# alonbebchuk/GNN-Pretraining

Hardware: AMD Instinct MI355X
Metric: pretrain graphs/sec (s4 multi-task) (higher is better)
Workload: dtype fp32; 1 GPU; s4 (NFM+LP+NC+GC+GP) pre-training step, 4 domains x 8 synthetic ENZYMES-shaped graphs per rank (input dims 7/4/37/21, hidden 256, 5 GIN layers), PCGrad + clip + AdamW; global_batch_graphs=32, parallelism=dp1, setup_steps=30, full=False, index_rng=reference, index_draws=native (csrc_host/hostdraw.cpp), cross_stream_sync=gates, ranks=1, devices_visible=1

## Files before the change

gnn_pretraining_amd/csrc/gemm_f32.hip:

```cpp
#include <algorithm>
#include <cstdlib>
#include <cstring>
#include <type_traits>

#include "gnnmp_internal.h"

namespace {

using gmp::f32x16;

constexpr int BK_DEFAULT = 32;
constexpr int THREADS = 256;

template <int R, bool KMAJOR, int BK>
struct TileLoader {
    static constexpr int NV = R * BK / 4 / THREADS;
    float4 v[NV];

    __device__ __forceinline__ void load(const float* __restrict__ P, int64_t ld, int64_t r0, int64_t rtot, int64_t k0,
                                         int64_t K, bool vec, int t) {
#pragma unroll
        for (int s = 0; s < NV; ++s) {
            const int f = t + s * THREADS;
            float4 x = make_float4(0.f, 0.f, 0.f, 0.f);
// ... 243 lines not shown
                    if (g.accumulate) v += out[row * ldo + col];
                    if (EPI) {
                        if (g.resid) v += g.resid[row * g.ldr + col];
                        if (g.scale) v = v * sc + sh;
                    }
                    if (g.relu) v = fmaxf(v, 0.f);
                }
                out[row * ldo + col] = v;
            }
        }
}

__global__ __launch_bounds__(256) void splitk_reduce_kernel(GemmArgs g) {
    const int64_t total = g.M * g.N;
    for (int64_t i = (int64_t)blockIdx.x * 256 + threadIdx.x; i < total; i += (int64_t)gridDim.x * 256) {
        float s = 0.f;
        for (int z = 0; z < g.splitk; ++z) s += g.partial[(int64_t)z * total + i];
        const int64_t row = i / g.N, col = i % g.N;
        float v = g.alpha * s + (g.bias ? g.bias[col] : 0.f);
        if (g.accumulate) v += g.C[row * g.ldc + col];
        if (g.resid) v += g.resid[row * g.ldr + col];
        if (g.scale) v = v * g.scale[col] + g.shift[col];
        if (g.relu) v = fmaxf(v, 0.f);
        g.C[row * g.ldc + col] = v;
    }
}

template <bool VEC>
__global__ __launch_bounds__(256) void grouped_reduce_kernel(const GemmArgs g) {
    const int grp = blockIdx.y;
    const int64_t total = g.M * g.N;
    if (VEC) {
        const int64_t quads = total / 4, mq = (g.M + 3) / 4;
        for (int64_t q = (int64_t)blockIdx.x * 256 + threadIdx.x; q < quads + mq; q += (int64_t)gridDim.x * 256) {
            if (q < quads) {
                const float* base = g.gpart + (int64_t)grp * g.gsplit * total + 4 * q;
                float4 s = make_float4(0.f, 0.f, 0.f, 0.f);
                for (int z0 = 0; z0 < g.gsplit; z0 += 8) {
                    float4 v[8];
#pragma unroll
                    for (int u = 0; u < 8; ++u)
                        v[u] = z0 + u < g.gsplit ? *reinterpret_cast<const float4*>(base + (int64_t)(z0 + u) * total) : make_float4(0.f, 0.f, 0.f, 0.f);
#pragma unroll
                    for (int u = 0; u < 8; ++u)
                        if (z0 + u < g.gsplit) { s.x += v[u].x; s.y += v[u].y; s.z += v[u].z; s.w += v[u].w; }
                }
                const int64_t i = 4 * q;
                *reinterpret_cast<float4*>(g.C + g.coff[grp] + (i / g.N) * g.ldc + i % g.N) = make_float4(g.alpha * s.x, g.alpha * s.y, g.alpha * s.z, g.alpha * s.w);
            } else if (g.asum) {
                for (int64_t m = 4 * (q - quads); m < g.M && m < 4 * (q - quads) + 4; ++m) {
                    float s = 0.f;
                    for (int z = 0; z < g.gsplit; ++z) s += g.gasum_part[((int64_t)grp * g.gsplit + z) * g.M + m];
                    g.asum[g.asumoff[grp] + m] = s;
                }
            }
        }
        return;
    }
    for (int64_t i = (int64_t)blockIdx.x * 256 + threadIdx.x; i < total + g.M; i += (int64_t)gridDim.x * 256) {
        float s = 0.f;
        if (i < total) {
            for (int z = 0; z < g.gsplit; ++z) s += g.gpart[((int64_t)grp * g.gsplit + z) * total + i];
            g.C[g.coff[grp] + (i / g.N) * g.ldc + i % g.N] = g.alpha * s;
        } else if (g.asum) {
            const int64_t m = i - total;
            for (int z = 0; z < g.gsplit; ++z) s += g.gasum_part[((int64_t)grp * g.gsplit + z) * g.M + m];
            g.asum[g.asumoff[grp] + m] = s;
        }
    }
}

inline void launch_grouped_reduce(const GemmArgs& g, int groups, hipStream_t st) {
    bool vec = g.N % 4 == 0 && g.ldc % 4 == 0 && (((uintptr_t)g.C | (uintptr_t)g.gpart) & 15) == 0;
    for (int i = 0; i < groups && vec; ++i) vec = g.coff[i] % 4 == 0;
    if (vec) {
        const int blocks = (int)std::min<int64_t>((g.M * g.N / 4 + (g.M + 3) / 4 + 255) / 256, 256);
        hipLaunchKernelGGL(grouped_reduce_kernel<true>, dim3(blocks, groups), dim3(256), 0, st, g);
    } else {
        const int blocks = (int)std::min<int64_t>((g.M * g.N + g.M + 255) / 256, 256);
        hipLaunchKernelGGL(grouped_reduce_kernel<false>, dim3(blocks, groups), dim3(256), 0, st, g);
    }
}

constexpr int CS_ROWS = 256;
__global__ __launch_bounds__(256) void colsum_partial_kernel(const float* __restrict__ A, float* __restrict__ part,
                                                             int64_t M, int64_t N, int64_t lda) {
    __shared__ float sh[4][64];
    const int c = threadIdx.x % 64, rl = threadIdx.x / 64;
    const int64_t col = (int64_t)blockIdx.x * 64 + c;
    const int64_t r0 = (int64_t)blockIdx.y * CS_ROWS, r1 = r0 + CS_ROWS < M ? r0 + CS_ROWS : M;
    float s = 0.f;
    if (col < N)
        for (int64_t r = r0 + rl; r < r1; r += 4) s += A[r * lda + col];
    sh[rl][c] = s;
    __syncthreads();
    if (rl == 0 && col < N) part[(int64_t)blockIdx.y * N + col] = (sh[0][c] + sh[1][c]) + (sh[2][c] + sh[3][c]);
}
__global__ __launch_bounds__(256) void colsum_final_kernel(const float* __restrict__ part, float* __restrict__ out,
                                                           int64_t nparts, int64_t N, int accumulate) {
    const int64_t col = (int64_t)blockIdx.x * 256 + threadIdx.x;
    if (col >= N) return;
    float s = 0.f;
    for (int64_t p = 0; p < nparts; ++p) s += part[p * N + col];
    out[col] = accumulate ? out[col] + s : s;
}

inline bool aligned16(const void* p) { return ((uintptr_t)p & 15) == 0; }

template <int BK>
bool fast_ok(int mode, const GemmArgs& g, int64_t min_rows) {
    if (!g.vecA || !g.vecB) return false;
    if (mode == GMP_GEMM_NT) return g.K % BK == 0 && g.K > 0 && min_rows >= 1 && g.N >= 1;
    if (mode == GMP_GEMM_NN) return g.K % BK == 0 && g.K > 0 && min_rows >= 1 && g.N % 4 == 0 && g.N >= 4;
    return g.M % 4 == 0 && g.M >= 4 && g.N % 4 == 0 && g.N >= 4;
}

template <int BM, int BN, int BK = BK_DEFAULT>
void launch_mode(int mode, const GemmArgs& g, dim3 grid, hipStream_t st, bool fast = false) {
#define GMP_GEMM_LAUNCH(AK, BKM)                                                                                    \
    do {                                                                                                           \
        if (fast) hipLaunchKernelGGL((gemm_kernel<BM, BN, AK, BKM, BK, true>), grid, dim3(THREADS), 0, st, g);      \
        else hipLaunchKernelGGL((gemm_kernel<BM, BN, AK, BKM, BK, false>), grid, dim3(THREADS), 0, st, g);          \
    } while (0)
    switch (mode) {
        case GMP_GEMM_NT:
            if (g.scale || g.resid) {
                if (fast) hipLaunchKernelGGL((gemm_kernel<BM, BN, false, false, BK, true, true>), grid, dim3(THREADS), 0, st, g);
                else hipLaunchKernelGGL((gemm_kernel<BM, BN, false, false, BK, false, true>), grid, dim3(THREADS), 0, st, g);
                break;
            }
            GMP_GEMM_LAUNCH(false, false);
            break;
        case GMP_GEMM_NN: GMP_GEMM_LAUNCH(false, true); break;
        default:          GMP_GEMM_LAUNCH(true, true); break;
    }
#undef GMP_GEMM_LAUNCH
}

constexpr int PIPE_TILES[4][2] = {{2, 2}, {1, 2}, {2, 1}, {1, 1}};

template <int TM, int TN, bool A_KC, bool B_KC, int STAGES, int BUFS = STAGES, bool EPI = false>
int launch_pipe_cfg(const GemmArgs& g, int tiles_m, int tiles_n, int z, hipStream_t st) {
    if constexpr (!EPI && A_KC && B_KC) {
        if (g.scale || g.resid) return launch_pipe_cfg<TM, TN, A_KC, B_KC, STAGES, BUFS, true>(g, tiles_m, tiles_n, z, st);
    }
    using C = g2::Cfg<TM, TN, A_KC, B_KC, STAGES, BUFS>;
    auto kern = g2::gemm_pipe_kernel<TM, TN, A_KC, B_KC, STAGES, BUFS, EPI>;
    static std::atomic<uint64_t> attr_set{0};
    if (int rc = gmp::reserve_lds(attr_set, reinterpret_cast<const void*>(kern), C::LDS_BYTES, "gemm_pipe")) return rc;
    hipLaunchKernelGGL(kern, dim3((unsigned)(tiles_m * tiles_n), 1, (unsigned)z), dim3(g2::THREADS), C::LDS_BYTES, st, g, tiles_m, tiles_n);
    return gmp::check_launch("gemm_pipe_kernel");
}

template <bool KC, int GEN>
int launch_pipe_gen(const GemmArgs& g, int64_t rows, int z, hipStream_t st) {
    using C = g2::Cfg<1, 1, KC, KC, 4, 4>;
    auto kern = g2::gemm_pipe_kernel<1, 1, KC, KC, 4, 4, false, GEN>;
    static std::atomic<uint64_t> attr_set{0};
    if (int rc = gmp::reserve_lds(attr_set, reinterpret_cast<const void*>(kern), C::LDS_BYTES, "gemm_pipe (generated operand)")) return rc;
    const int tiles_m = (int)((rows + 63) / 64), tiles_n = (int)((g.N + 63) / 64);
    hipLaunchKernelGGL(kern, dim3((unsigned)(tiles_m * tiles_n), 1, (unsigned)z), dim3(g2::THREADS), C::LDS_BYTES, st, g, tiles_m, tiles_n);
    return gmp::check_launch("gemm_pipe_kernel (generated operand)");
}

template <bool A_KC, bool B_KC>
int launch_pipe_tile(int tile, const GemmArgs& g, int64_t rows, int z, hipStream_t st) {
    const int TMs = PIPE_TILES[tile][0], TNs = PIPE_TILES[tile][1];
    const int tiles_m = (int)((rows + 64 * TMs - 1) / (64 * TMs)), tiles_n = (int)((g.N + 64 * TNs - 1) / (64 * TNs));
    const char* e = getenv("GMP_GEMM_PIPE_STAGES");
    const int deep = e ? atoi(e) : 0;
    switch (tile) {
        case 0: return launch_pipe_cfg<2, 2, A_KC, B_KC, 4>(g, tiles_m, tiles_n, z, st);
        case 1: return deep == 3 ? launch_pipe_cfg<1, 2, A_KC, B_KC, 3>(g, tiles_m, tiles_n, z, st)
                                 : launch_pipe_cfg<1, 2, A_KC, B_KC, 4>(g, tiles_m, tiles_n, z, st);
        case 2: return deep == 3 ? launch_pipe_cfg<2, 1, A_KC, B_KC, 3>(g, tiles_m, tiles_n, z, st)
                                 : launch_pipe_cfg<2, 1, A_KC, B_KC, 4>(g, tiles_m, tiles_n, z, st);
        default: return deep == 3 ? launch_pipe_cfg<1, 1, A_KC, B_KC, 3>(g, tiles_m, tiles_n, z, st)
                      : deep == 32 ? launch_pipe_cfg<1, 1, A_KC, B_KC, 3, 2>(g, tiles_m, tiles_n, z, st)
                                   : launch_pipe_cfg<1, 1, A_KC, B_KC, 4>(g, tiles_m, tiles_n, z, st);
    }
}

int launch_pipe(int mode, int tile, const GemmArgs& g_in, int64_t rows, int z, hipStream_t st) {
    const GemmArgs& g = g_in;
    if (mode == GMP_GEMM_NT) return launch_pipe_tile<true, true>(tile, g, rows, z, st);
    if (mode == GMP_GEMM_NN) return launch_pipe_tile<true, false>(tile, g, rows, z, st);
    return launch_pipe_tile<false, false>(tile, g, rows, z, st);
}

inline bool pipe_enabled() {
    const char* e = getenv("GMP_GEMM_IMPL");
    return !(e && !strcmp(e, "old"));
}
inline int64_t pipe_min_rows() { return 1024; }
inline int pipe_forced_tile() {
    const char* e = getenv("GMP_GEMM_PIPE_TILE");
    return e ? atoi(e) : -1;
}

int pipe_pick_tile(int64_t rows, int64_t N, int64_t z) {
    (void)rows; (void)N; (void)z;
    if (pipe_forced_tile() >= 0 && pipe_forced_tile() < 4) return pipe_forced_tile();
    return 3;
}

bool pipe_ok(int mode, const GemmArgs& g) {
    if (!pipe_enabled() || !g.vecA || !g.vecB) return false;
    if (mode == GMP_GEMM_NT) return g.K >= 64 && g.K % g2::BK == 0;
    if (mode == GMP_GEMM_NN) return g.K >= 64 && g.K % g2::BK == 0 && g.N % 4 == 0 && g.N >= 4;
    return g.M % 4 == 0 && g.M >= 4 && g.N % 4 == 0 && g.N >= 4;
}

inline bool takes_pipe(int mode, const GemmArgs& g) {
    return mode != GMP_GEMM_TN && g.M >= pipe_min_rows() && g.N >= 64 && pipe_ok(mode, g) && (g.splitk == 1 || g.N % 4 == 0);
}

}

namespace gmp {
void signal_on_next_gemm(int32_t* flag, int value) {
    t_sig_flag = (int*)flag;
    t_sig_value = value;
}
bool signal_pending() { return t_sig_flag != nullptr; }
}

extern "C" int gmp_gate_open_by_next_gemm(int32_t* flag, int value) {
    gmp::signal_on_next_gemm(flag, value);
    return GMP_OK;
}
extern "C" int gmp_gate_open_pending(void) { return gmp::signal_pending() ? 1 : 0; }

extern "C" size_t gmp_gemm_f32_workspace_bytes(int mode, int64_t M, int64_t N, int64_t K) {
    if (M <= 0 || N <= 0 || K <= 0) return 0;
    const int64_t tiles = ((M + 63) / 64) * ((N + 63) / 64);
    if (tiles >= 256 || K < 8 * BK_DEFAULT) return 0;
    const int64_t steps = (K + BK_DEFAULT - 1) / BK_DEFAULT;
    if (mode != GMP_GEMM_TN && !((tiles <= 96 && steps >= 32) || (tiles <= 48 && steps >= 16))) return 0;
    int64_t sk = (512 + tiles - 1) / tiles;
    if (sk > steps / 2) sk = steps / 2;
    if (sk < 2) return 0;
    return (size_t)sk * M * N * sizeof(float);
}

extern "C" int gmp_gemm_f32(int mode, const float* A, const float* B, const float* bias, float* C, int64_t M, int64_t N,
                            int64_t K, int64_t lda, int64_t ldb, int64_t ldc, float alpha, int accumulate, int relu,
                            void* workspace, size_t workspace_bytes, gmp_stream_t stream) {
    return gmp::gemm_f32_epilogue(mode, A, B, bias, C, M, N, K, lda, ldb, ldc, alpha, accumulate, relu, nullptr, nullptr, nullptr, 0, workspace,
                                  workspace_bytes, stream);
}

int gmp::gemm_f32_epilogue(int mode, const float* A, const float* B, const float* bias, float* C, int64_t M, int64_t N, int64_t K, int64_t lda,
                           int64_t ldb, int64_t ldc, float alpha, int accumulate, int relu, const float* scale, const float* shift,
                           const float* resid, int64_t ldr, void* workspace, size_t workspace_bytes, gmp_stream_t stream) {
    const bool epi = scale || shift || resid;
    if (epi && (mode != GMP_GEMM_NT || !scale != !shift || (resid && ldr < N))) return gmp::fail(GMP_ERR_ARG, "gemm: affine epilogue operands");
    if (mode < 0 || mode > 2) return gmp::fail(GMP_ERR_ARG, "gemm: mode %d", mode);
    if (M < 0 || N < 0 || K < 0) return gmp::fail(GMP_ERR_ARG, "gemm: negative size");
    if (M == 0 || N == 0) return GMP_OK;
    if (!C || (K > 0 && (!A || !B))) return gmp::fail(GMP_ERR_ARG, "gemm: null pointer");
    const int64_t need_lda = mode == GMP_GEMM_TN ? M : K, need_ldb = mode == GMP_GEMM_NT ? K : N;
    if (lda < need_lda || ldb < need_ldb || ldc < N)
        return gmp::fail(GMP_ERR_ARG, "gemm: leading dims (%lld,%lld,%lld) too small for M=%lld N=%lld K=%lld mode %d",
                         (long long)lda, (long long)ldb, (long long)ldc, (long long)M, (long long)N, (long long)K, mode);
    hipStream_t st = (hipStream_t)stream;
    GemmArgs g{A, B, bias, C, M, N, K, lda, ldb, ldc, alpha, accumulate, relu, 1, nullptr,
               (lda % 4 == 0) && aligned16(A), (ldb % 4 == 0) && aligned16(B)};
    if (!epi) take_signal(g);
    g.vecC = (ldc % 4 == 0) && aligned16(C);
    if (epi) {
        g.scale = scale; g.shift = shift; g.resid = resid; g.ldr = ldr;
        if (N % 4 || !aligned16(bias) || !aligned16(scale) || !aligned16(shift) || !aligned16(resid) || ldr % 4) g.vecC = 0;
    }
    const size_t want = gmp_gemm_f32_workspace_bytes(mode, M, N, K);
    if (want && workspace && workspace_bytes >= want) {
        g.splitk = (int)(want / ((size_t)M * N * sizeof(float)));
        g.partial = (float*)workspace;
    }
    static const int forced = getenv("GMP_GEMM_TILE") ? atoi(getenv("GMP_GEMM_TILE")) : -1;
    const int64_t t128 = ((M + 127) / 128) * ((N + 127) / 128), t12864 = ((M + 127) / 128) * ((N + 63) / 64);
    int tile = 0;
    (void)t12864;
    if (g.splitk == 1) tile = t128 >= 4096 ? 2 : 0;
    if (forced >= 0 && forced <= 2 && g.splitk == 1) tile = forced;
    if (takes_pipe(mode, g)) {
        if (g.splitk == 1) return launch_pipe(mode, pipe_pick_tile(M, N, 1), g, M, 1, st);
        if (int rc = launch_pipe(mode, pipe_pick_tile(M, N, 1), g, M, g.splitk, st)) return rc;
        const int blocks = (int)std::min<int64_t>((M * N + 255) / 256, 2048);
        hipLaunchKernelGGL(splitk_reduce_kernel, dim3(blocks), dim3(256), 0, st, g);
        return gmp::check_launch("splitk_reduce_kernel");
    }
    static const bool nofast = getenv("GMP_GEMM_NOFAST") != nullptr;
    const bool fast = !nofast && fast_ok<BK_DEFAULT>(mode, g, M);
    if (tile == 2) launch_mode<128, 128>(mode, g, dim3((unsigned)((N + 127) / 128), (unsigned)((M + 127) / 128), 1), st, fast);
    else if (tile == 1) launch_mode<128, 64>(mode, g, dim3((unsigned)((N + 63) / 64), (unsigned)((M + 127) / 128), 1), st, fast);
    else if (forced == 3) launch_mode<64, 64, 64>(mode, g, dim3((unsigned)((N + 63) / 64), (unsigned)((M + 63) / 64), (unsigned)g.splitk), st, !nofast && fast_ok<64>(mode, g, M));
    else if (forced == 4) launch_mode<64, 64, 16>(mode, g, dim3((unsigned)((N + 63) / 64), (unsigned)((M + 63) / 64), (unsigned)g.splitk), st, fast);
    else launch_mode<64, 64>(mode, g, dim3((unsigned)((N + 63) / 64), (unsigned)((M + 63) / 64), (unsigned)g.splitk), st, fast);
    if (int rc = gmp::check_launch("gemm_kernel")) return rc;
    if (g.splitk > 1) {
        int blocks = (int)std::min<int64_t>((M * N + 255) / 256, 2048);
        hipLaunchKernelGGL(splitk_reduce_kernel, dim3(blocks), dim3(256), 0, st, g);
        return gmp::check_launch("splitk_reduce_kernel");
    }
    return GMP_OK;
}

namespace {
struct GenOperand { const float* h; const int64_t* edges; int64_t N, K; };
int grouped_impl(int mode, const float* A, const float* B, const float* bias, float* C, int groups, const int32_t* group_rows_host,
                 const int64_t* b_off_host, const int64_t* bias_off_host, const int64_t* c_off_host, float* a_colsum,
                 const int64_t* a_colsum_off_host, int64_t M_tn, int64_t N, int64_t K, int64_t lda, int64_t ldb, int64_t ldc, float alpha,
                 int accumulate, int relu, void* workspace, size_t workspace_bytes, gmp_stream_t stream, const GenOperand* gen);
}

// ... 222 lines not shown
```

gnn_pretraining_amd/csrc/gemm_pipe.h:

```cpp
#pragma once

namespace g2 {

using gmp::f32x16;
typedef __attribute__((address_space(3))) void lds_void;
typedef const __attribute__((address_space(1))) void glb_void;

constexpr int BK = 32;
constexpr int THREADS = 256;
#ifndef GMP_PIPE_SCHED
#define GMP_PIPE_SCHED 1
#endif


__device__ __forceinline__ void glds16(const float* src, unsigned lds_addr) {
    unsigned keep;
    asm volatile("s_mov_b32 %0, m0\n\ts_mov_b32 m0, %2\n\ts_nop 0\n\tglobal_load_lds_dwordx4 %1, off\n\ts_mov_b32 m0, %0"
                 : "=&s"(keep)
                 : "v"(src), "s"(lds_addr)
                 : "memory");
}
__device__ __forceinline__ unsigned lds_address(const char* p) {
    return __builtin_amdgcn_readfirstlane((unsigned)(size_t)(const __attribute__((address_space(3))) char*)p);
}

template <int R, bool KC>
struct Operand {
    static constexpr int BYTES = R * BK * 4;
    static constexpr int INSTR = BYTES / 1024;
    static constexpr int PER_WAVE = INSTR / 4;
    static constexpr int LPR = R / 4;

    const float* p[PER_WAVE];
    int64_t step;

    __device__ __forceinline__ void init(const float* __restrict__ P, int64_t ld, int64_t r0, int64_t rtot, int64_t k0, int lane, int wave,
                                         bool wrap = false) {
#pragma unroll
        for (int i = 0; i < PER_WAVE; ++i) {
            const int ii = wave + 4 * i;
            if (KC) {
                const int row = ii * 8 + (lane >> 3);
                const int chunk = (lane & 7) ^ ((row >> 1) & 7);
                int64_t gr = r0 + row;
                gr = gr < rtot ? gr : (wrap ? r0 + row % (int)(rtot - r0) : rtot - 1);
                p[i] = P + gr * ld + k0 + 4 * chunk;
            } else {
                const int k = ii * (64 / LPR) + lane / LPR, q = lane % LPR;
                int64_t gr = r0 + 4 * q;
                gr = gr + 3 < rtot ? gr : rtot - 4;
                p[i] = P + (k0 + k) * ld + gr;
            }
        }
        step = KC ? BK : BK * ld;
    }

    __device__ __forceinline__ void issue(unsigned stage_addr, int wave) {
#pragma unroll
        for (int i = 0; i < PER_WAVE; ++i) {
            glds16(p[i], stage_addr + (wave + 4 * i) * 1024);
            p[i] += step;
        }
    }

    __device__ __forceinline__ void issue_tail(unsigned stage_addr, int wave, int lane, int64_t klen, int64_t ld) {
#pragma unroll
        for (int i = 0; i < PER_WAVE; ++i) {
            const int k = (wave + 4 * i) * (64 / LPR) + lane / LPR;
            const int64_t back = k < klen ? 0 : (int64_t)(k - (klen - 1)) * ld;
            glds16(p[i] - back, stage_addr + (wave + 4 * i) * 1024);
        }
    }
};

template <int R, bool KC>
__device__ __forceinline__ void read_frag(const char* tile, int rb, int g, int l31, int half, float (&f)[4]) {
    if (KC) {
        const int r = rb + l31;
        const float4 v = *reinterpret_cast<const float4*>(tile + r * 128 + ((((2 * g + half) ^ ((r >> 1) & 7))) << 4));
        f[0] = v.x; f[1] = v.y; f[2] = v.z; f[3] = v.w;
    } else {
#pragma unroll
        for (int j = 0; j < 4; ++j) f[j] = *reinterpret_cast<const float*>(tile + ((8 * g + 4 * half + j) * R + rb + l31) * 4);
    }
}

template <int TM, int TN, bool A_KC, bool B_KC, int STAGES, int BUFS = STAGES>
struct Cfg {
    static_assert(BUFS == STAGES || BUFS == STAGES - 1, "buffers: one per stage of the schedule, or one less (early free)");
    static_assert(BUFS >= 2, "at least two buffers");
    static constexpr int BM = 64 * TM, BN = 64 * TN;
    using OA = Operand<BM, A_KC>;
    using OB = Operand<BN, B_KC>;
    static constexpr int STAGE_BYTES = OA::BYTES + OB::BYTES;
    static constexpr int LDS_BYTES = BUFS * STAGE_BYTES;
    static constexpr int LOADS = OA::PER_WAVE + OB::PER_WAVE;
};

template <int N>
__device__ __forceinline__ void wait_vmcnt() {
    asm volatile("s_waitcnt vmcnt(%0)" ::"n"(N) : "memory");
}

template <int TM, int TN, bool A_KC, bool B_KC, int STAGES>
__device__ __forceinline__ void read_sub(const char* st, int g, int wm, int wn, int l31, int half, float (&fa)[TM][4], float (&fb)[TN][4]) {
    using C = Cfg<TM, TN, A_KC, B_KC, STAGES>;
#pragma unroll
    for (int i = 0; i < TM; ++i) read_frag<C::BM, A_KC>(st, wm * (C::BM / 2) + 32 * i, g, l31, half, fa[i]);
#pragma unroll
    for (int j = 0; j < TN; ++j) read_frag<C::BN, B_KC>(st + C::OA::BYTES, wn * (C::BN / 2) + 32 * j, g, l31, half, fb[j]);
}

template <int TM, int TN, bool TAIL>
__device__ __forceinline__ void mfma_sub(f32x16 (&acc)[TM][TN], const float (&fa)[TM][4], const float (&fb)[TN][4], int g, int half, int klen) {
#pragma unroll
    for (int j4 = 0; j4 < 4; ++j4) {
        const bool dead = TAIL && (8 * g + 4 * half + j4 >= klen);
#pragma unroll
        for (int i = 0; i < TM; ++i)
#pragma unroll
            for (int j = 0; j < TN; ++j) {
                const float a = dead ? 0.f : fa[i][j4];
                const float b = dead ? 0.f : fb[j][j4];
                acc[i][j] = __builtin_amdgcn_mfma_f32_32x32x2f32(a, b, acc[i][j], 0, 0, 0);
            }
    }
}

template <int NREADS, int NMFMA>
__device__ __forceinline__ void sched_sub() {
#if GMP_PIPE_SCHED == 1
    __builtin_amdgcn_sched_group_barrier(0x008, 1, 0);
    __builtin_amdgcn_sched_group_barrier(0x100, NREADS, 0);
    __builtin_amdgcn_sched_group_barrier(0x008, NMFMA - 1, 0);
#endif
}

template <int TM, int TN, bool A_KC, bool B_KC, int STAGES, int BUFS = STAGES, bool EPI = false, int GEN = 0>
__global__ __launch_bounds__(THREADS) void gemm_pipe_kernel(const GemmArgs g, int tiles_m, int tiles_n) {
    using C = Cfg<TM, TN, A_KC, B_KC, STAGES, BUFS>;
    constexpr bool EARLY = BUFS < STAGES;
    constexpr bool IS_TN = !A_KC && !B_KC;
    constexpr bool GEN_A = GEN == 1, GEN_B = GEN == 2;
    static_assert(GEN == 0 || (GEN_A && A_KC && B_KC) || (GEN_B && IS_TN), "generated operand: A of the NT form or B of the TN form");
    static_assert(GEN == 0 || (!EARLY && !EPI), "generated operand: one buffer per stage, plain epilogue");
    constexpr int DMA_LOADS = (GEN_A ? 0 : C::OA::PER_WAVE) + (GEN_B ? 0 : C::OB::PER_WAVE);
    extern __shared__ __attribute__((aligned(16))) char smem[];

    const int t = threadIdx.x, lane = t & 63;
    const int wave = __builtin_amdgcn_readfirstlane(t >> 6);
    const int wm = wave >> 1, wn = wave & 1, l31 = lane & 31, half = lane >> 5;
    if (g.sig_flag && t == 0 && blockIdx.x == 0 && blockIdx.z == 0)
        __hip_atomic_store(g.sig_flag, g.sig_value, __ATOMIC_RELEASE, __HIP_MEMORY_SCOPE_AGENT);

    int bid = blockIdx.x;
    {
        const int nwg = gridDim.x, q = nwg >> 3, r = nwg & 7, xcd = bid & 7;
        bid = (xcd < r ? xcd * (q + 1) : r * (q + 1) + (xcd - r) * q) + (bid >> 3);
    }
    const int tile_m = bid / tiles_n, tile_n = bid - tile_m * tiles_n;
    int64_t m0 = (int64_t)tile_m * C::BM;
    const int64_t n0 = (int64_t)tile_n * C::BN;

    const float* __restrict__ Bp = g.B;
    const float* __restrict__ biasp = g.bias;
    float* Cp = g.C;
    int64_t Mrows = g.M;
    int64_t kbeg = 0, kend = g.K;
    if (g.groups > 0) {
        const int grp = IS_TN ? blockIdx.z / g.gsplit : blockIdx.z;
        if (IS_TN) {
            kbeg = g.grow[grp];
            kend = g.grow[grp + 1];
            if (g.gsplit > 1) {
                const int64_t steps = (kend - kbeg + BK - 1) / BK, per = (steps + g.gsplit - 1) / g.gsplit;
                kbeg += (int64_t)(blockIdx.z % g.gsplit) * per * BK;
                kend = kbeg + per * BK < kend ? kbeg + per * BK : kend;
                Cp = g.gpart + (int64_t)blockIdx.z * g.M * g.N;
            } else {
                Cp += g.coff[grp];
            }
        } else {
            m0 += g.grow[grp];
            Mrows = g.grow[grp + 1];
            if (m0 >= Mrows) return;
            Bp += g.boff[grp];
            if (biasp) biasp += g.biasoff[grp];
        }
    }
    const bool ksplit = !IS_TN && g.groups == 0 && g.splitk > 1;
    if (ksplit) {
        const int64_t steps = g.K / BK, per = (steps + g.splitk - 1) / g.splitk;
        kbeg = (int64_t)blockIdx.z * per * BK;
        kend = kbeg + per * BK < g.K ? kbeg + per * BK : g.K;
        Cp = g.partial + (int64_t)blockIdx.z * g.M * g.N;
    }
    const int64_t klen_total = kend > kbeg ? kend - kbeg : 0;
    const int nfull = (int)(klen_total / BK);
    const int ktail = (int)(klen_total - (int64_t)nfull * BK);
    const int nsteps = nfull + (ktail ? 1 : 0);

    f32x16 acc[TM][TN];
#pragma unroll
    for (int i = 0; i < TM; ++i)
#pragma unroll
        for (int j = 0; j < TN; ++j)
#pragma unroll
            for (int r = 0; r < 16; ++r) acc[i][j][r] = 0.f;

    typename C::OA la;
    typename C::OB lb;
    if (nsteps > 0) {
        if (!GEN_A) la.init(g.A, g.lda, m0, Mrows, kbeg, lane, wave);
        if (!GEN_B) lb.init(Bp, g.ldb, n0, g.N, kbeg, lane, wave);
    }
    auto stage_ptr = [&](int s) -> char* { return smem + (s % BUFS) * C::STAGE_BYTES; };
    const unsigned lds0 = lds_address(smem);
    auto issue = [&](int s) {
        const unsigned sp = lds0 + (s % BUFS) * C::STAGE_BYTES;
        if (IS_TN && ktail && s == nfull) {
            if (!GEN_A) la.issue_tail(sp, wave, lane, ktail, g.lda);
            if (!GEN_B) lb.issue_tail(sp + C::OA::BYTES, wave, lane, ktail, g.ldb);
        } else {
            if (!GEN_A) la.issue(sp, wave);
            if (!GEN_B) lb.issue(sp + C::OA::BYTES, wave);
        }
    };
    constexpr int NS = GEN_A ? C::OA::PER_WAVE : C::OB::PER_WAVE;
    constexpr int LPRB = C::OB::LPR;
    const float4* __restrict__ gh4 = reinterpret_cast<const float4*>(g.gen_h);
    int64_t gia[NS], gib[NS];
    float4 gvs[NS], gvd[NS];
    auto gen_idx = [&](int s) {
#pragma unroll
        for (int i = 0; i < NS; ++i) {
            const int ii = wave + 4 * i;
            int64_t r;
            if (GEN_A) {
                r = m0 + ii * 8 + (lane >> 3);
                r = r < Mrows ? r : Mrows - 1;
            } else {
                r = kbeg + (int64_t)s * BK + ii * (64 / LPRB) + lane / LPRB;
                r = r < kend ? r : kend - 1;
            }
            gia[i] = g.gen_edges[r];
            gib[i] = g.gen_edges[g.gen_K + r];
        }
    };
    auto gen_load = [&](int s) {
#pragma unroll
        for (int i = 0; i < NS; ++i) {
            const int ii = wave + 4 * i;
            int cq;
            if (GEN_A) {
                const int row = ii * 8 + (lane >> 3);
                cq = 8 * (s & 7) + ((lane & 7) ^ ((row >> 1) & 7));
            } else {
                cq = (int)(n0 & 255) / 4 + lane % LPRB;
            }
            const bool oka = gia[i] >= 0 && gia[i] < g.gen_N, okb = gib[i] >= 0 && gib[i] < g.gen_N;
            float4 sv = make_float4(0.f, 0.f, 0.f, 0.f), dv = sv;
            if (oka) sv = gh4[gia[i] * 64 + cq];
            if (okb) dv = gh4[gib[i] * 64 + cq];
            gvs[i] = sv;
            gvd[i] = dv;
        }
    };
    auto gen_store = [&](int s) {
        const int third = GEN_A ? (s >> 3) : (int)(n0 >> 8);
        char* dst = stage_ptr(s) + (GEN_B ? C::OA::BYTES : 0);
#pragma unroll
        for (int i = 0; i < NS; ++i) {
            const float4 a = gvs[i], b = gvd[i];
            float4 v;
            if (third == 0) v = make_float4(a.x + b.x, a.y + b.y, a.z + b.z, a.w + b.w);
            else if (third == 1) v = make_float4(a.x * b.x, a.y * b.y, a.z * b.z, a.w * b.w);
            else v = make_float4(fabsf(a.x - b.x), fabsf(a.y - b.y), fabsf(a.z - b.z), fabsf(a.w - b.w));
            *reinterpret_cast<float4*>(dst + (wave + 4 * i) * 1024 + lane * 16) = v;
        }
    };
    if (GEN != 0 && nsteps > 0) {
        gen_idx(0);
        gen_load(0);
        gen_store(0);
        if (nsteps > 1) {
            if (GEN_B) gen_idx(1);
            gen_load(1);
        }
        if (GEN_B && nsteps > 2) gen_idx(2);
    }
#pragma unroll
    for (int s = 0; s < STAGES - 1; ++s)
        if (s < nsteps) issue(s);

    const bool want_asum = IS_TN && g.groups > 0 && g.asum != nullptr && tile_n == 0;
    constexpr int QUADS = C::BM / 4, KSL = THREADS / QUADS, KPER = BK / KSL;
    float4 colacc = make_float4(0.f, 0.f, 0.f, 0.f);

    float fa0[TM][4], fa1[TM][4], fb0[TN][4], fb1[TN][4];
    constexpr int NREADS = (A_KC ? TM : 4 * TM) + (B_KC ? TN : 4 * TN), NMFMA = 4 * TM * TN;
    if (nsteps > 0) {
        if (STAGES >= 4 && nsteps >= 3) wait_vmcnt<2 * DMA_LOADS>();
        else if (STAGES >= 3 && nsteps >= 2) wait_vmcnt<DMA_LOADS>();
        else wait_vmcnt<0>();
        if (GEN != 0) asm volatile("s_waitcnt lgkmcnt(0)" ::: "memory");
        __builtin_amdgcn_s_barrier();
        read_sub<TM, TN, A_KC, B_KC, STAGES>(stage_ptr(0), 0, wm, wn, l31, half, fa0, fb0);
    }
    auto step = [&](int s, auto tailc) {
        constexpr bool TAIL = decltype(tailc)::value;
        const char* st = stage_ptr(s);
        const int klen = TAIL ? ktail : BK;
        if (want_asum) {
            const int mq = t % QUADS, ks = t / QUADS;
#pragma unroll
            for (int kk = 0; kk < KPER; ++kk) {
                const int k = ks * KPER + kk;
                if (!TAIL || k < klen) {
                    const float4 v = *reinterpret_cast<const float4*>(st + (k * C::BM + 4 * mq) * 4);
                    colacc.x += v.x; colacc.y += v.y; colacc.z += v.z; colacc.w += v.w;
                }
            }
        }
        read_sub<TM, TN, A_KC, B_KC, STAGES>(st, 1, wm, wn, l31, half, fa1, fb1);
        mfma_sub<TM, TN, TAIL>(acc, fa0, fb0, 0, half, klen);
        sched_sub<NREADS, NMFMA>();
        read_sub<TM, TN, A_KC, B_KC, STAGES>(st, 2, wm, wn, l31, half, fa0, fb0);
        mfma_sub<TM, TN, TAIL>(acc, fa1, fb1, 1, half, klen);
        sched_sub<NREADS, NMFMA>();
        read_sub<TM, TN, A_KC, B_KC, STAGES>(st, 3, wm, wn, l31, half, fa1, fb1);
        mfma_sub<TM, TN, TAIL>(acc, fa0, fb0, 2, half, klen);
        sched_sub<NREADS, NMFMA>();
        if (s + 1 < nsteps) {
            if (STAGES >= 4 && s + 2 < nsteps) wait_vmcnt<DMA_LOADS>();
            else wait_vmcnt<0>();
            if (EARLY) asm volatile("s_waitcnt lgkmcnt(0)" ::: "memory");
            if (GEN != 0) {
                gen_store(s + 1);
                asm volatile("s_waitcnt lgkmcnt(0)" ::: "memory");
            }
            __builtin_amdgcn_s_barrier();
            if (GEN != 0 && s + 2 < nsteps) {
                gen_load(s + 2);
                if (GEN_B && s + 3 < nsteps) gen_idx(s + 3);
            }
            if (s + STAGES - 1 < nsteps) issue(s + STAGES - 1);
            read_sub<TM, TN, A_KC, B_KC, STAGES>(stage_ptr(s + 1), 0, wm, wn, l31, half, fa0, fb0);
        }
        mfma_sub<TM, TN, TAIL>(acc, fa1, fb1, 3, half, klen);
    };
    for (int s = 0; s < nfull; ++s) step(s, std::false_type{});
    if (ktail) step(nfull, std::true_type{});

    if (want_asum) {
        __builtin_amdgcn_s_barrier();
        float4* red = reinterpret_cast<float4*>(smem);
        red[t] = colacc;
        asm volatile("s_waitcnt lgkmcnt(0)" ::: "memory");
        __builtin_amdgcn_s_barrier();
        if (t < C::BM && m0 + t < g.M) {
            const float* rf = reinterpret_cast<const float*>(smem);
            float sum = 0.f;
#pragma unroll
            for (int ks = 0; ks < KSL; ++ks) sum += rf[(ks * QUADS + (t >> 2)) * 4 + (t & 3)];
            if (g.gsplit > 1) g.gasum_part[(int64_t)blockIdx.z * g.M + m0 + t] = sum;
            else g.asum[g.asumoff[blockIdx.z] + m0 + t] = sum;
        }
    }

    float* out = Cp;
    int64_t ldo = g.ldc;
    const bool partial = (IS_TN && g.groups > 0 && g.gsplit > 1) || ksplit;
    if (partial) ldo = g.N;
    constexpr int WR = 32 * TM, WC = 32 * TN;
    const int64_t row0 = m0 + wm * WR, col0 = n0 + wn * WC;
    if (g.vecC || partial) {
        __builtin_amdgcn_s_barrier();
        float* tile = reinterpret_cast<float*>(smem) + wave * (WR * WC);
#pragma unroll
        for (int i = 0; i < TM; ++i)
#pragma unroll
            for (int j = 0; j < TN; ++j)
#pragma unroll
                for (int r = 0; r < 16; ++r)
                    tile[gmp::acc_row(r, half, i * 32) * WC + j * 32 + l31] = acc[i][j][r];
        constexpr int LR = WC / 4, RPI = 64 / LR;
        const int c4 = lane % LR, rsub = lane / LR;
        const int64_t col = col0 + 4 * c4;
        float4 bv = make_float4(0.f, 0.f, 0.f, 0.f);
        if (!partial && biasp) {
            if (col + 3 < g.N) bv = *reinterpret_cast<const float4*>(biasp + col);
            else {
                if (col < g.N) bv.x = biasp[col];
                if (col + 1 < g.N) bv.y = biasp[col + 1];
                if (col + 2 < g.N) bv.z = biasp[col + 2];
            }
        }
        float4 sc = make_float4(1.f, 1.f, 1.f, 1.f), sh = make_float4(0.f, 0.f, 0.f, 0.f);
        if (EPI && !partial && g.scale && col + 3 < g.N) {
            sc = *reinterpret_cast<const float4*>(g.scale + col);
            sh = *reinterpret_cast<const float4*>(g.shift + col);
        }
#pragma unroll
        for (int q = 0; q < WR / RPI; ++q) {
            const int rl = q * RPI + rsub;
            float4 v = *reinterpret_cast<const float4*>(tile + rl * WC + 4 * c4);
            const int64_t row = row0 + rl;
            if (row >= Mrows || col >= g.N) continue;
            float* o = out + row * ldo + col;
            const bool full = col + 3 < g.N;
            if (!partial) {
                v.x = g.alpha * v.x + bv.x; v.y = g.alpha * v.y + bv.y; v.z = g.alpha * v.z + bv.z; v.w = g.alpha * v.w + bv.w;
                if (g.accumulate) {
                    if (full) {
                        const float4 c = *reinterpret_cast<const float4*>(o);
                        v.x += c.x; v.y += c.y; v.z += c.z; v.w += c.w;
                    } else {
                        v.x += o[0];
                        if (col + 1 < g.N) v.y += o[1];
                        if (col + 2 < g.N) v.z += o[2];
                    }
                }
                if (EPI) {
                    if (g.resid) {
                        const float4 c = *reinterpret_cast<const float4*>(g.resid + row * g.ldr + col);
                        v.x += c.x; v.y += c.y; v.z += c.z; v.w += c.w;
                    }
                    if (g.scale) { v.x = v.x * sc.x + sh.x; v.y = v.y * sc.y + sh.y; v.z = v.z * sc.z + sh.z; v.w = v.w * sc.w + sh.w; }
                }
                if (g.relu) { v.x = fmaxf(v.x, 0.f); v.y = fmaxf(v.y, 0.f); v.z = fmaxf(v.z, 0.f); v.w = fmaxf(v.w, 0.f); }
            }
            if (full) {
                *reinterpret_cast<float4*>(o) = v;
            }
            else {
                o[0] = v.x;
                if (col + 1 < g.N) o[1] = v.y;
                if (col + 2 < g.N) o[2] = v.z;
            }
        }
        return;
    }
#pragma unroll
    for (int i = 0; i < TM; ++i)
#pragma unroll
        for (int j = 0; j < TN; ++j) {
            const int64_t col = col0 + j * 32 + l31;
            if (col >= g.N) continue;
            const float bv = (!partial && biasp) ? biasp[col] : 0.f;
            const float sc = (EPI && g.scale) ? g.scale[col] : 1.f, sh = (EPI && g.scale) ? g.shift[col] : 0.f;
#pragma unroll
            for (int r = 0; r < 16; ++r) {
                const int64_t row = gmp::acc_row(r, half, row0 + i * 32);
                if (row >= Mrows) continue;
                float v = g.alpha * acc[i][j][r] + bv;
                if (g.accumulate) v += out[row * ldo + col];
                if (EPI) {
                    if (g.resid) v += g.resid[row * g.ldr + col];
                    if (g.scale) v = v * sc + sh;
                }
                if (g.relu) v = fmaxf(v, 0.f);
                out[row * ldo + col] = v;
            }
        }
}

struct LpFoldArgs {
    const float* gy1;
    const float* w0;
    const float* h;
    const int64_t* edges;
    float* ghs;
    float* ghd;
    int64_t N, K;
    float alpha;
    int* sig_flag;
    int sig_value;
};

__device__ __forceinline__ float lp_sgn(float v) { return (float)((v > 0.f) - (v < 0.f)); }

__global__ __launch_bounds__(THREADS) void lp_bwd_fold_kernel(const LpFoldArgs g, int tiles_m) {
    constexpr int STAGES = 4;
    using C = Cfg<1, 1, true, false, STAGES>;
    constexpr int F = 256, KS = F / BK, NSTEPS = 3 * KS, TILES_N = F / C::BN;
    static_assert(4 * 3 * 32 * 32 * 4 <= C::LDS_BYTES, "the epilogue turns three sub-tiles per wave through the ring");
    extern __shared__ __attribute__((aligned(16))) char smem[];

    const int t = threadIdx.x, lane = t & 63;
    const int wave = __builtin_amdgcn_readfirstlane(t >> 6);
    const int wm = wave >> 1, wn = wave & 1, l31 = lane & 31, half = lane >> 5;
    if (g.sig_flag && t == 0 && blockIdx.x == 0)
        __hip_atomic_store(g.sig_flag, g.sig_value, __ATOMIC_RELEASE, __HIP_MEMORY_SCOPE_AGENT);

    int bid = blockIdx.x;
    {
        const int nwg = gridDim.x, q = nwg >> 3, r = nwg & 7, xcd = bid & 7;
        bid = (xcd < r ? xcd * (q + 1) : r * (q + 1) + (xcd - r) * q) + (bid >> 3);
    }
    const int tile_m = bid / TILES_N, tile_n = bid - tile_m * TILES_N;
    if (tile_m >= tiles_m) return;
    const int64_t m0 = (int64_t)tile_m * C::BM;
    const int c0 = tile_n * C::BN;

    f32x16 acc[3][1][1];
// ... 90 lines not shown
```

Baseline: 24270 graphs/s.

## Stream generated LP operand rows via async LDS DMA and combine in registers

The generated-operand GEMM path (link-prediction features built as sum/product/abs-diff of two gathered node rows) no longer loads gathered rows into registers and combines them before storing to LDS. Both source and destination rows are now copied straight into LDS with global_load_lds, and edge indices for the B form are prefetched the same way. The sum/product/distance is computed per fragment after the LDS read, just before the MFMA. This removes the register-staged load/store and its extra lgkmcnt waits from the pipeline. In exchange it doubles the LDS reads and per-stage LDS footprint for the generated operand. It also defaults to a 4-stage/3-buffer ring selectable by an environment variable.

```diff
diff --git a/gnn_pretraining_amd/csrc/gemm_f32.hip b/gnn_pretraining_amd/csrc/gemm_f32.hip
--- a/gnn_pretraining_amd/csrc/gemm_f32.hip
+++ b/gnn_pretraining_amd/csrc/gemm_f32.hip
@@ -419,15 +419,25 @@
     return gmp::check_launch("gemm_pipe_kernel");
 }
 
+template <bool KC, int GEN, int STAGES, int BUFS>
+int launch_pipe_gen_ring(const GemmArgs& g, int64_t rows, int z, hipStream_t st) {
+    using C = g2::Cfg<1, 1, KC, KC, STAGES, BUFS>;
+    constexpr int LDS_BYTES = BUFS * (C::STAGE_BYTES + (GEN == 1 ? C::OA::BYTES : C::OB::BYTES)) + (GEN == 2 ? STAGES * 2 * g2::BK * 8 : 0);
+    auto kern = g2::gemm_pipe_kernel<1, 1, KC, KC, STAGES, BUFS, false, GEN>;
+    static std::atomic<uint64_t> attr_set{0};
+    if (int rc = gmp::reserve_lds(attr_set, reinterpret_cast<const void*>(kern), LDS_BYTES, "gemm_pipe (generated operand)")) return rc;
+    const int tiles_m = (int)((rows + 63) / 64), tiles_n = (int)((g.N + 63) / 64);
+    hipLaunchKernelGGL(kern, dim3((unsigned)(tiles_m * tiles_n), 1, (unsigned)z), dim3(g2::THREADS), LDS_BYTES, st, g, tiles_m, tiles_n);
+    return gmp::check_launch("gemm_pipe_kernel (generated operand)");
+}
+
 template <bool KC, int GEN>
 int launch_pipe_gen(const GemmArgs& g, int64_t rows, int z, hipStream_t st) {
-    using C = g2::Cfg<1, 1, KC, KC, 4, 4>;
-    auto kern = g2::gemm_pipe_kernel<1, 1, KC, KC, 4, 4, false, GEN>;
-    static std::atomic<uint64_t> attr_set{0};
-    if (int rc = gmp::reserve_lds(attr_set, reinterpret_cast<const void*>(kern), C::LDS_BYTES, "gemm_pipe (generated operand)")) return rc;
-    const int tiles_m = (int)((rows + 63) / 64), tiles_n = (int)((g.N + 63) / 64);
-    hipLaunchKernelGGL(kern, dim3((unsigned)(tiles_m * tiles_n), 1, (unsigned)z), dim3(g2::THREADS), C::LDS_BYTES, st, g, tiles_m, tiles_n);
-    return gmp::check_launch("gemm_pipe_kernel (generated operand)");
+    const char* e = getenv("GMP_LP_GEN_RING");
+    const int ring = e ? atoi(e) : 43;
+    if (ring == 44) return launch_pipe_gen_ring<KC, GEN, 4, 4>(g, rows, z, st);
+    if (ring == 33) return launch_pipe_gen_ring<KC, GEN, 3, 3>(g, rows, z, st);
+    return launch_pipe_gen_ring<KC, GEN, 4, 3>(g, rows, z, st);
 }
 
 template <bool A_KC, bool B_KC>
diff --git a/gnn_pretraining_amd/csrc/gemm_pipe.h b/gnn_pretraining_amd/csrc/gemm_pipe.h
--- a/gnn_pretraining_amd/csrc/gemm_pipe.h
+++ b/gnn_pretraining_amd/csrc/gemm_pipe.h
@@ -16,6 +16,13 @@
 __device__ __forceinline__ void glds16(const float* src, unsigned lds_addr) {
     unsigned keep;
     asm volatile("s_mov_b32 %0, m0\n\ts_mov_b32 m0, %2\n\ts_nop 0\n\tglobal_load_lds_dwordx4 %1, off\n\ts_mov_b32 m0, %0"
+                 : "=&s"(keep)
+                 : "v"(src), "s"(lds_addr)
+                 : "memory");
+}
+__device__ __forceinline__ void glds4(const float* src, unsigned lds_addr) {
+    unsigned keep;
+    asm volatile("s_mov_b32 %0, m0\n\ts_mov_b32 m0, %2\n\ts_nop 0\n\tglobal_load_lds_dword %1, off\n\ts_mov_b32 m0, %0"
                  : "=&s"(keep)
                  : "v"(src), "s"(lds_addr)
                  : "memory");
@@ -136,6 +143,16 @@
 #endif
 }
 
+static __device__ __attribute__((aligned(16))) float lp_zero_row[256];
+
+__device__ __forceinline__ void lp_third(int third, const float (&a)[4], const float (&b)[4], float (&v)[4]) {
+#pragma unroll
+    for (int j = 0; j < 4; ++j) {
+        const float sum = a[j] + b[j], prod = a[j] * b[j], dist = fabsf(a[j] - b[j]);
+        v[j] = third == 0 ? sum : third == 1 ? prod : dist;
+    }
+}
+
 template <int TM, int TN, bool A_KC, bool B_KC, int STAGES, int BUFS = STAGES, bool EPI = false, int GEN = 0>
 __global__ __launch_bounds__(THREADS) void gemm_pipe_kernel(const GemmArgs g, int tiles_m, int tiles_n) {
     using C = Cfg<TM, TN, A_KC, B_KC, STAGES, BUFS>;
@@ -143,8 +160,11 @@
     constexpr bool IS_TN = !A_KC && !B_KC;
     constexpr bool GEN_A = GEN == 1, GEN_B = GEN == 2;
     static_assert(GEN == 0 || (GEN_A && A_KC && B_KC) || (GEN_B && IS_TN), "generated operand: A of the NT form or B of the TN form");
-    static_assert(GEN == 0 || (!EARLY && !EPI), "generated operand: one buffer per stage, plain epilogue");
-    constexpr int DMA_LOADS = (GEN_A ? 0 : C::OA::PER_WAVE) + (GEN_B ? 0 : C::OB::PER_WAVE);
+    static_assert(GEN == 0 || (TM == 1 && TN == 1 && !EPI), "generated operand: 64 x 64 tile, plain epilogue");
+    constexpr int GEN_BYTES = GEN_A ? C::OA::BYTES : GEN_B ? C::OB::BYTES : 0;
+    constexpr int STAGE_BYTES = C::STAGE_BYTES + GEN_BYTES;
+    constexpr int B_OFF = C::OA::BYTES + (GEN_A ? GEN_BYTES : 0);
+    constexpr int DMA_LOADS = C::LOADS + (GEN_A ? C::OA::PER_WAVE : GEN_B ? C::OB::PER_WAVE : 0);
     extern __shared__ __attribute__((aligned(16))) char smem[];
 
     const int t = threadIdx.x, lane = t & 63;
@@ -214,103 +234,148 @@
         if (!GEN_A) la.init(g.A, g.lda, m0, Mrows, kbeg, lane, wave);
         if (!GEN_B) lb.init(Bp, g.ldb, n0, g.N, kbeg, lane, wave);
     }
-    auto stage_ptr = [&](int s) -> char* { return smem + (s % BUFS) * C::STAGE_BYTES; };
+    auto stage_ptr = [&](int s) -> char* { return smem + (s % BUFS) * STAGE_BYTES; };
     const unsigned lds0 = lds_address(smem);
-    auto issue = [&](int s) {
-        const unsigned sp = lds0 + (s % BUFS) * C::STAGE_BYTES;
-        if (IS_TN && ktail && s == nfull) {
-            if (!GEN_A) la.issue_tail(sp, wave, lane, ktail, g.lda);
-            if (!GEN_B) lb.issue_tail(sp + C::OA::BYTES, wave, lane, ktail, g.ldb);
+    constexpr int NS = GEN_A ? C::OA::PER_WAVE : C::OB::PER_WAVE;
+    const float* zrow = nullptr;
+    if constexpr (GEN != 0) {
+        zrow = lp_zero_row;
+        asm volatile("" : "+s"(zrow));
+    }
+    auto gen_row = [&](int64_t idx) -> const float* {
+        return idx >= 0 && idx < g.gen_N ? g.gen_h + idx * 256 : zrow;
+    };
+    const float *gps[NS], *gpd[NS];
+    if constexpr (GEN_A) {
+        if (nsteps > 0) {
+#pragma unroll
+            for (int i = 0; i < NS; ++i) {
+                const int row = (wave + 4 * i) * 8 + (lane >> 3);
+                const int chunk = (lane & 7) ^ ((row >> 1) & 7);
+                int64_t r = m0 + row;
+                r = r < Mrows ? r : Mrows - 1;
+                gps[i] = gen_row(g.gen_edges[r]) + 4 * chunk;
+                gpd[i] = gen_row(g.gen_edges[g.gen_K + r]) + 4 * chunk;
+            }
+        }
+    }
+    static_assert(!GEN_B || NS == 2, "generated B: two DMA slots per wave (64 columns)");
+    constexpr int IDX_BYTES = 2 * BK * 8, IDX_OFF = BUFS * STAGE_BYTES;
+    auto idx_issue = [&](int s) {
+        if (wave < 2) {
+            int64_t r = kbeg + (int64_t)s * BK + (lane >> 1);
+            r = r < kend ? r : kend - 1;
+            glds4(reinterpret_cast<const float*>(g.gen_edges + wave * g.gen_K + r) + (lane & 1), lds0 + IDX_OFF + (s % STAGES) * IDX_BYTES + wave * 256);
+        }
+    };
+    auto issue = [&](int s, bool ahead) {
+        const unsigned sp = lds0 + (s % BUFS) * STAGE_BYTES;
+        if constexpr (GEN == 0) {
+            if (IS_TN && ktail && s == nfull) {
+                la.issue_tail(sp, wave, lane, ktail, g.lda);
+                lb.issue_tail(sp + C::OA::BYTES, wave, lane, ktail, g.ldb);
+            } else {
+                la.issue(sp, wave);
+                lb.issue(sp + C::OA::BYTES, wave);
+            }
+            return;
+        }
+        const bool tail = IS_TN && ktail && s == nfull;
+        const float *ps[2], *pd[2];
+        if constexpr (GEN_B) {
+            const int64_t* ix = reinterpret_cast<const int64_t*>(smem + IDX_OFF + (s % STAGES) * IDX_BYTES);
+            const int64_t col = (n0 & 255) + 4 * (lane & 15);
+#pragma unroll
+            for (int i = 0; i < 2; ++i) {
+                const int k = (wave + 4 * i) * 4 + (lane >> 4);
+                ps[i] = gen_row(ix[k]) + col;
+                pd[i] = gen_row(ix[BK + k]) + col;
+            }
+            if (ahead && s + 1 < nsteps) idx_issue(s + 1);
+        }
+        if constexpr (GEN_A) {
+#pragma unroll
+            for (int i = 0; i < NS; ++i) {
+                glds16(gps[i], sp + (wave + 4 * i) * 1024);
+                glds16(gpd[i], sp + GEN_BYTES + (wave + 4 * i) * 1024);
+                gps[i] += BK;
+                gpd[i] += BK;
+            }
+            if ((s & 7) == 7) {
+#pragma unroll
+                for (int i = 0; i < NS; ++i) { gps[i] -= 256; gpd[i] -= 256; }
+            }
         } else {
-            if (!GEN_A) la.issue(sp, wave);
-            if (!GEN_B) lb.issue(sp + C::OA::BYTES, wave);
-        }
-    };
-    constexpr int NS = GEN_A ? C::OA::PER_WAVE : C::OB::PER_WAVE;
-    constexpr int LPRB = C::OB::LPR;
-    const float4* __restrict__ gh4 = reinterpret_cast<const float4*>(g.gen_h);
-    int64_t gia[NS], gib[NS];
-    float4 gvs[NS], gvd[NS];
-    auto gen_idx = [&](int s) {
-#pragma unroll
-        for (int i = 0; i < NS; ++i) {
-            const int ii = wave + 4 * i;
-            int64_t r;
-            if (GEN_A) {
-                r = m0 + ii * 8 + (lane >> 3);
-                r = r < Mrows ? r : Mrows - 1;
-            } else {
-                r = kbeg + (int64_t)s * BK + ii * (64 / LPRB) + lane / LPRB;
-                r = r < kend ? r : kend - 1;
-            }
-            gia[i] = g.gen_edges[r];
-            gib[i] = g.gen_edges[g.gen_K + r];
-        }
-    };
-    auto gen_load = [&](int s) {
-#pragma unroll
-        for (int i = 0; i < NS; ++i) {
-            const int ii = wave + 4 * i;
-            int cq;
-            if (GEN_A) {
-                const int row = ii * 8 + (lane >> 3);
-                cq = 8 * (s & 7) + ((lane & 7) ^ ((row >> 1) & 7));
-            } else {
-                cq = (int)(n0 & 255) / 4 + lane % LPRB;
-            }
-            const bool oka = gia[i] >= 0 && gia[i] < g.gen_N, okb = gib[i] >= 0 && gib[i] < g.gen_N;
-            float4 sv = make_float4(0.f, 0.f, 0.f, 0.f), dv = sv;
-            if (oka) sv = gh4[gia[i] * 64 + cq];
-            if (okb) dv = gh4[gib[i] * 64 + cq];
-            gvs[i] = sv;
-            gvd[i] = dv;
-        }
-    };
-    auto gen_store = [&](int s) {
-        const int third = GEN_A ? (s >> 3) : (int)(n0 >> 8);
-        char* dst = stage_ptr(s) + (GEN_B ? C::OA::BYTES : 0);
-#pragma unroll
-        for (int i = 0; i < NS; ++i) {
-            const float4 a = gvs[i], b = gvd[i];
-            float4 v;
-            if (third == 0) v = make_float4(a.x + b.x, a.y + b.y, a.z + b.z, a.w + b.w);
-            else if (third == 1) v = make_float4(a.x * b.x, a.y * b.y, a.z * b.z, a.w * b.w);
-            else v = make_float4(fabsf(a.x - b.x), fabsf(a.y - b.y), fabsf(a.z - b.z), fabsf(a.w - b.w));
-            *reinterpret_cast<float4*>(dst + (wave + 4 * i) * 1024 + lane * 16) = v;
-        }
-    };
-    if (GEN != 0 && nsteps > 0) {
-        gen_idx(0);
-        gen_load(0);
-        gen_store(0);
-        if (nsteps > 1) {
-            if (GEN_B) gen_idx(1);
-            gen_load(1);
-        }
-        if (GEN_B && nsteps > 2) gen_idx(2);
+            if (tail) la.issue_tail(sp, wave, lane, ktail, g.lda);
+            else la.issue(sp, wave);
+        }
+        if constexpr (GEN_B) {
+#pragma unroll
+            for (int i = 0; i < 2; ++i) {
+                glds16(ps[i], sp + B_OFF + (wave + 4 * i) * 1024);
+                glds16(pd[i], sp + B_OFF + GEN_BYTES + (wave + 4 * i) * 1024);
+            }
+        } else {
+            if (tail) lb.issue_tail(sp + B_OFF, wave, lane, ktail, g.ldb);
+            else lb.issue(sp + B_OFF, wave);
+        }
+    };
+    if constexpr (GEN_B) {
+#pragma unroll
+        for (int s = 0; s < STAGES; ++s)
+            if (s < nsteps) idx_issue(s);
+        wait_vmcnt<0>();
+        __builtin_amdgcn_s_barrier();
     }
 #pragma unroll
     for (int s = 0; s < STAGES - 1; ++s)
-        if (s < nsteps) issue(s);
+        if (s < nsteps) issue(s, false);
 
     const bool want_asum = IS_TN && g.groups > 0 && g.asum != nullptr && tile_n == 0;
     constexpr int QUADS = C::BM / 4, KSL = THREADS / QUADS, KPER = BK / KSL;
     float4 colacc = make_float4(0.f, 0.f, 0.f, 0.f);
 
     float fa0[TM][4], fa1[TM][4], fb0[TN][4], fb1[TN][4];
-    constexpr int NREADS = (A_KC ? TM : 4 * TM) + (B_KC ? TN : 4 * TN), NMFMA = 4 * TM * TN;
+    float xs0[4], xd0[4], xs1[4], xd1[4];
+    constexpr int NREADS = (A_KC ? TM : 4 * TM) * (GEN_A ? 2 : 1) + (B_KC ? TN : 4 * TN) * (GEN_B ? 2 : 1), NMFMA = 4 * TM * TN;
+    auto rd = [&](const char* st, int gs, float (&fa)[TM][4], float (&fb)[TN][4], float (&xs)[4], float (&xd)[4]) {
+        if constexpr (GEN_A) {
+            read_frag<C::BM, true>(st, wm * 32, gs, l31, half, xs);
+            read_frag<C::BM, true>(st + GEN_BYTES, wm * 32, gs, l31, half, xd);
+            read_frag<C::BN, true>(st + B_OFF, wn * 32, gs, l31, half, fb[0]);
+        } else {
+            read_frag<C::BM, false>(st, wm * 32, gs, l31, half, fa[0]);
+            read_frag<C::BN, false>(st + B_OFF, wn * 32, gs, l31, half, xs);
+            read_frag<C::BN, false>(st + B_OFF + GEN_BYTES, wn * 32, gs, l31, half, xd);
+        }
+    };
+    auto mm = [&](auto tailc, int gs, int third, float (&fa)[TM][4], float (&fb)[TN][4], const float (&xs)[4], const float (&xd)[4], int klen) {
+        if constexpr (GEN_A) lp_third(third, xs, xd, fa[0]);
+        else lp_third(third, xs, xd, fb[0]);
+        mfma_sub<TM, TN, decltype(tailc)::value>(acc, fa, fb, gs, half, klen);
+    };
+#define G2_READ(st, gs, fa, fb, xs, xd)                                                                 \
+    do {                                                                                                \
+        if constexpr (GEN == 0) read_sub<TM, TN, A_KC, B_KC, STAGES>(st, gs, wm, wn, l31, half, fa, fb); \
+        else rd(st, gs, fa, fb, xs, xd);                                                                \
+    } while (0)
+#define G2_MFMA(gs, fa, fb, xs, xd)                                                     \
+    do {                                                                                \
+        if constexpr (GEN == 0) mfma_sub<TM, TN, TAIL>(acc, fa, fb, gs, half, klen);    \
+        else mm(tailc, gs, third, fa, fb, xs, xd, klen);                                \
+    } while (0)
     if (nsteps > 0) {
         if (STAGES >= 4 && nsteps >= 3) wait_vmcnt<2 * DMA_LOADS>();
         else if (STAGES >= 3 && nsteps >= 2) wait_vmcnt<DMA_LOADS>();
         else wait_vmcnt<0>();
-        if (GEN != 0) asm volatile("s_waitcnt lgkmcnt(0)" ::: "memory");
         __builtin_amdgcn_s_barrier();
-        read_sub<TM, TN, A_KC, B_KC, STAGES>(stage_ptr(0), 0, wm, wn, l31, half, fa0, fb0);
+        G2_READ(stage_ptr(0), 0, fa0, fb0, xs0, xd0);
     }
     auto step = [&](int s, auto tailc) {
         constexpr bool TAIL = decltype(tailc)::value;
         const char* st = stage_ptr(s);
         const int klen = TAIL ? ktail : BK;
+        const int third = GEN_A ? (s >> 3) : (int)(n0 >> 8);
         if (want_asum) {
             const int mq = t % QUADS, ks = t / QUADS;
 #pragma unroll
@@ -322,35 +387,29 @@
                 }
             }
         }
-        read_sub<TM, TN, A_KC, B_KC, STAGES>(st, 1, wm, wn, l31, half, fa1, fb1);
-        mfma_sub<TM, TN, TAIL>(acc, fa0, fb0, 0, half, klen);
+        G2_READ(st, 1, fa1, fb1, xs1, xd1);
+        G2_MFMA(0, fa0, fb0, xs0, xd0);
         sched_sub<NREADS, NMFMA>();
-        read_sub<TM, TN, A_KC, B_KC, STAGES>(st, 2, wm, wn, l31, half, fa0, fb0);
-        mfma_sub<TM, TN, TAIL>(acc, fa1, fb1, 1, half, klen);
+        G2_READ(st, 2, fa0, fb0, xs0, xd0);
+        G2_MFMA(1, fa1, fb1, xs1, xd1);
         sched_sub<NREADS, NMFMA>();
-        read_sub<TM, TN, A_KC, B_KC, STAGES>(st, 3, wm, wn, l31, half, fa1, fb1);
-        mfma_sub<TM, TN, TAIL>(acc, fa0, fb0, 2, half, klen);
+        G2_READ(st, 3, fa1, fb1, xs1, xd1);
+        G2_MFMA(2, fa0, fb0, xs0, xd0);
         sched_sub<NREADS, NMFMA>();
         if (s + 1 < nsteps) {
             if (STAGES >= 4 && s + 2 < nsteps) wait_vmcnt<DMA_LOADS>();
             else wait_vmcnt<0>();
             if (EARLY) asm volatile("s_waitcnt lgkmcnt(0)" ::: "memory");
-            if (GEN != 0) {
-                gen_store(s + 1);
-                asm volatile("s_waitcnt lgkmcnt(0)" ::: "memory");
-            }
             __builtin_amdgcn_s_barrier();
-            if (GEN != 0 && s + 2 < nsteps) {
-                gen_load(s + 2);
-                if (GEN_B && s + 3 < nsteps) gen_idx(s + 3);
-            }
-            if (s + STAGES - 1 < nsteps) issue(s + STAGES - 1);
-            read_sub<TM, TN, A_KC, B_KC, STAGES>(stage_ptr(s + 1), 0, wm, wn, l31, half, fa0, fb0);
-        }
-        mfma_sub<TM, TN, TAIL>(acc, fa1, fb1, 3, half, klen);
+            if (s + STAGES - 1 < nsteps) issue(s + STAGES - 1, true);
+            G2_READ(stage_ptr(s + 1), 0, fa0, fb0, xs0, xd0);
+        }
+        G2_MFMA(3, fa1, fb1, xs1, xd1);
     };
     for (int s = 0; s < nfull; ++s) step(s, std::false_type{});
     if (ktail) step(nfull, std::true_type{});
+#undef G2_READ
+#undef G2_MFMA
 
     if (want_asum) {
         __builtin_amdgcn_s_barrier();
```

Result: slower. 23790 graphs/s (-2.0%).
